# sadhusamik/speech_recognition_tools

Hardware: AMD Instinct MI355X
Metric: audio-hours/sec FDLP featurized (16 kHz, 80-band) (higher is better)
Workload: dtype f64; 1 GPU; wsj_si284_4s_batches; params=wsj, scp_entries_total=1024, batches_in_flight=4, utts_per_batch=1024, nfilters=80, order=150, coeff_num=100, coeff_range=0,100, fbank=cochlear,1,1,1,2.5,1, add_noise=clean, parallelism=scp-shard x1 (contiguous split_scp shards, no collective)

## Files before the change

### speech_recognition_tools_amd/csrc/fdlp_autocorr.hip

```cpp
#include <hip/hip_runtime.h>
#include <math.h>

#include <algorithm>
#include <type_traits>
#include <stdint.h>
#include <stdlib.h>

#include "fdlp_device.h"

namespace fdlp {

constexpr int kAcChunk = 256;
constexpr int kAcRing = 512;
constexpr int kAcPer = kAcChunk / 64;
constexpr int kMaxWrapLags = 256;

template <int NT>
__global__ __launch_bounds__(64, 4) void autocorr_kernel(DevConsts c, const double* __restrict__ dct,
                                                      const double* __restrict__ dense,
                                                      double* __restrict__ rout) {
  static_assert(16 * NT <= kAcChunk, "window halo must fit one chunk");
  constexpr int G = 2;
  constexpr int kEpi = (16 * G + 15) * 17;
  constexpr int kStage = 2 * kAcRing;
  constexpr int kLds = kStage > kEpi ? kStage : kEpi;
  constexpr int NLPL = (16 * NT + 63) / 64;
  __shared__ double xs[kLds];

  const int item = blockIdx.x;
  const int lane = threadIdx.x;
  const int N = c.N;
  int lo, hi;
  const double* drow;
  const double* wrow = nullptr;
  if (dense) {
    lo = 0;
    hi = N;
    drow = dense + (int64_t)item * N;
  } else {
    const int f = item / c.B, j = item % c.B;
    lo = c.lo[j];
    hi = c.hi[j];
    drow = dct + (int64_t)f * N;
    wrow = c.fbank + (int64_t)j * N;
  }
  const int i_lane = lane & 15;
  const int kk_lane = lane >> 4;

  dbl4 acc[NT];
#pragma unroll
  for (int t = 0; t < NT; ++t) acc[t] = dbl4{0.0, 0.0, 0.0, 0.0};

  const int span = hi - lo;
  const int nsteps = (span + 63) / 64;
  const int nchunks = (nsteps + kAcPer - 1) / kAcPer;
  double dv[kAcPer], wv[kAcPer];
  auto fetch = [&](int ch) {
#pragma unroll
    for (int q = 0; q < kAcPer; ++q) {
      int pos = lo + kAcChunk * ch + 64 * q + lane;
      if (pos >= N) pos -= N;
      const bool ok = pos >= lo && pos < hi;
      dv[q] = ok ? drow[pos] : 0.0;
      wv[q] = ok ? (wrow ? wrow[pos] : 1.0) : 0.0;
    }
  };
  auto store = [&](int ch) {
#pragma unroll
    for (int q = 0; q < kAcPer; ++q) {
      const int slot = (kAcChunk * ch + 64 * q + lane) & (kAcRing - 1);
      const double x = wv[q] * dv[q];
      xs[slot] = x;
      xs[slot + kAcRing] = x;
    }
  };
  if (nsteps > 0) {
    fetch(0);
    store(0);
    fetch(1);
    store(1);
    fetch(2);
  }
  __syncthreads();
  for (int ch = 0; ch < nchunks; ++ch) {
    const int s_end = min(kAcPer, nsteps - kAcPer * ch);
    const int rbase = (kAcChunk * ch) & (kAcRing - 1);
    for (int st = 0; st < s_end; ++st) {
      const double* w = xs + rbase + 64 * st + 16 * kk_lane + i_lane;
      const double a = w[0];
#pragma unroll
      for (int t = 0; t < NT; ++t)
        acc[t] = __builtin_amdgcn_mfma_f64_16x16x4f64(a, w[16 * t], acc[t], 0, 0, 0);
    }
    __syncthreads();
    store(ch + 2);
    if (ch + 3 <= nchunks) fetch(ch + 3);
    __syncthreads();
  }

  const int nlags = c.nlags;
  double mine[NLPL];
#pragma unroll
  for (int q = 0; q < NLPL; ++q) mine[q] = 0.0;
  const int col = lane & 15;
  const int row0 = lane >> 4;
#pragma unroll
  for (int tg = 0; tg < NT; tg += G) {
    const int lag_base = 16 * tg - 15;
#pragma unroll
    for (int t = tg; t < tg + G && t < NT; ++t) {
#pragma unroll
      for (int r = 0; r < 4; ++r) {
        const int row = row0 + 4 * r;
        const int lag = 16 * t + col - row;
        xs[(lag - lag_base) * 17 + row] = acc[t][r];
      }
    }
    __syncthreads();
#pragma unroll
    for (int q = 0; q < NLPL; ++q) {
      const int L = lane + 64 * q;
      if (L < nlags && L >= lag_base && L < 16 * (tg + G)) {
        double s = 0.0;
        for (int i = 0; i < 16; ++i) {
          const int t = (L + i) >> 4;
          if (t >= tg && t < tg + G && t < NT) s += xs[(L - lag_base) * 17 + i];
        }
        mine[q] += s;
      }
    }
    __syncthreads();
  }
#pragma unroll
  for (int q = 0; q < NLPL; ++q) {
    const int L = lane + 64 * q;
    if (L < nlags && rout) rout[(int64_t)item * nlags + L] = mine[q];
  }
}


template <int NT, int G, int NLPL>
__device__ __forceinline__ void diag_sums(const dbl4* acc, double* ep, int nlags, int lane, double* mine) {
#pragma unroll
  for (int q = 0; q < NLPL; ++q) mine[q] = 0.0;
  const int col = lane & 15;
  const int row0 = lane >> 4;
#pragma unroll
  for (int tg = 0; tg < NT; tg += G) {
    const int lag_base = 16 * tg - 15;
#pragma unroll
    for (int t = tg; t < tg + G && t < NT; ++t) {
#pragma unroll
      for (int r = 0; r < 4; ++r) {
        const int row = row0 + 4 * r;
        ep[(16 * t + col - row - lag_base) * 17 + row] = acc[t][r];
      }
    }
    __syncthreads();
#pragma unroll
    for (int q = 0; q < NLPL; ++q) {
      const int L = lane + 64 * q;
      if (L < nlags && L >= lag_base && L < 16 * (tg + G)) {
        double s = 0.0;
#pragma unroll
        for (int i = 0; i < 16; ++i) {
          const int t = (L + i) >> 4;
          if (t >= tg && t < tg + G && t < NT) s += ep[(L - lag_base) * 17 + i];
        }
        mine[q] += s;
      }
    }
    __syncthreads();
  }
}

template <int NT, int LB, typename Emit>
__device__ __forceinline__ void diag_blocks(const dbl4* acc, double* ep, int nlags, int lane, Emit emit) {
  static_assert(LB == 32 || LB == 64, "lag block");
  constexpr int LPL = 64 / LB;
  constexpr int TPB = LB / 16;
  constexpr int NB = (16 * NT + LB - 1) / LB;
  const int col = lane & 15;
  const int row0 = lane >> 4;
  const int m = lane / LPL;
  const int part = lane % LPL;
#pragma unroll
  for (int g = 0; g < NB; ++g) {
    if (LB * g >= nlags) break;
#pragma unroll
    for (int u = 0; u <= TPB; ++u) {
      const int t = TPB * g + u;
#pragma unroll
      for (int r = 0; r < 4; ++r) {
        const int row = row0 + 4 * r;
        const double v = t < NT ? acc[t < NT ? t : 0][r] : 0.0;
        ep[(16 * u + col - row + 15) * 17 + row] = v;
      }
    }
    wave_lds_sync();
    const double* src = ep + (m + 15) * 17 + part * (16 / LPL);
    double v[16 / LPL];
#pragma unroll
    for (int i = 0; i < 16 / LPL; ++i) v[i] = src[i];
    double sum = 0.0;
#pragma unroll
    for (int i = 0; i < 16 / LPL; ++i) sum += v[i];
    if constexpr (LPL == 2) sum += dpp_f64<0xB1>(sum);
    const int L = LB * g + m;
    if (part == 0 && L < nlags) {
      if constexpr (std::is_invocable_v<Emit, int, int, double>) emit(g, L, sum);
      else emit(L, sum);
    }
    wave_lds_sync();
  }
}

template <int NT>
__device__ __forceinline__ void lag_step(dbl4* acc, const double* w, bool keep) {
  const double a = keep ? w[0] : 0.0;
#pragma unroll
  for (int t = 0; t < NT; ++t) acc[t] = __builtin_amdgcn_mfma_f64_16x16x4f64(a, w[16 * t], acc[t], 0, 0, 0);
}

template <int NT, int G, bool SNAP = true>
__global__ __launch_bounds__(64, 2) void ac_sweep_kernel(DevConsts c, const double* __restrict__ dct,
                                                         double* __restrict__ rlow, double* __restrict__ rup,
                                                         int nwork) {
  static_assert(16 * NT <= kAcChunk, "window halo must fit one chunk");
  constexpr int kEpi = (G + 31) * 17;
  __shared__ double xs[2 * kAcRing];
  __shared__ double ep[kEpi];

  const int w = xcd_item();
  if (w >= nwork) return;
  const int f = w >> 1;
  const int sk = w & 1;
  const int lane = threadIdx.x;
  const int N = c.N, B = c.B, nlags = c.nlags;
  const double* drow = dct + (int64_t)f * N;
  const double* ew = c.sk_e + (int64_t)sk * N;
  const SkSnap* snaps = c.sk_snap + sk * B;
  double* out = (sk == 0 ? rlow : rup) + (int64_t)f * B * nlags;
  const int T0 = ((N + kAcChunk - 1) / kAcChunk) * kAcChunk;
  const int bmin = c.sk_min[sk] >> 6;
  const int nblk = (T0 >> 6) - bmin;
  const int nchunks = (nblk + kAcPer - 1) / kAcPer;
  const int i_lane = lane & 15;
  const int kk_lane = lane >> 4;

  dbl4 acc[NT];
#pragma unroll
  for (int t = 0; t < NT; ++t) acc[t] = dbl4{0.0, 0.0, 0.0, 0.0};

  double dv[kAcPer], ev[kAcPer];
  auto fetch = [&](int ch) {
#pragma unroll
    for (int q = 0; q < kAcPer; ++q) {
      const int n = T0 - kAcChunk * (ch + 1) + 64 * q + lane;
      const bool ok = n >= 0 && n < N;
      const int m = ok ? (sk == 0 ? N - 1 - n : n) : 0;
      dv[q] = drow[m];
      ev[q] = ok ? ew[m] : 0.0;
    }
  };
  auto store = [&](int ch) {
#pragma unroll
    for (int q = 0; q < kAcPer; ++q) {
      const int slot = (T0 - kAcChunk * (ch + 1) + 64 * q + lane) & (kAcRing - 1);
      const double v = ev[q] * dv[q];
      xs[slot] = v;
      xs[slot + kAcRing] = v;
    }
  };
  extern __shared__ SkSnap tab[];
  for (int q = lane; q < B; q += 64) tab[q] = snaps[q];
  __syncthreads();
  int k = 0;
  SkSnap cur = tab[0];
  auto snapshot = [&]() {
    double* o = out + (int64_t)cur.band * nlags;
    const double K = cur.K;
    if constexpr (SNAP) {
      diag_blocks<NT, G>(acc, ep, nlags, lane, [&](int L, double v) { o[L] = K * v; });
    } else {
      double cs = 0.0;
#pragma unroll
      for (int t = 0; t < NT; ++t) cs += acc[t][0] + acc[t][1] + acc[t][2] + acc[t][3];
      if (lane < nlags) o[lane] = K * cs;
    }
    ++k;
    cur = k < B ? tab[k] : SkSnap{-1, 0, 0.0};
  };
  auto step = [&](int P, int lo, int hi) {
    const int pa = P + 16 * kk_lane + i_lane;
    lag_step<NT>(acc, xs + (P & (kAcRing - 1)) + 16 * kk_lane + i_lane, pa >= lo && pa < hi);
  };

#pragma unroll
  for (int q = 0; q < kAcPer; ++q) {
    const int slot = (T0 + 64 * q + lane) & (kAcRing - 1);
    xs[slot] = 0.0;
    xs[slot + kAcRing] = 0.0;
  }
  fetch(0);
  store(0);
  if (nchunks > 1) fetch(1);
  __syncthreads();
  for (int ch = 0; ch < nchunks; ++ch) {
    for (int q = kAcPer - 1; q >= 0; --q) {
      const int P = T0 - kAcChunk * (ch + 1) + 64 * q;
      if ((P >> 6) < bmin) break;
      int hiM = P + 64;
      while (k < B && cur.S >= hiM) snapshot();
      while (k < B && cur.S > P) {
        step(P, cur.S, hiM);
        hiM = cur.S;
        snapshot();
      }
      step(P, P, hiM);
    }
    __syncthreads();
    if (ch + 1 < nchunks) store(ch + 1);
    if (ch + 2 < nchunks) fetch(ch + 2);
    __syncthreads();
  }
  while (k < B) snapshot();
}

template <int NT, bool VS>
__global__ __launch_bounds__(64, 4) void ac_band_kernel(DevConsts c, const double* __restrict__ dct,
                                                        double* __restrict__ r, const double* __restrict__ rup,
                                                        const double* __restrict__ rflat,
                                                        const double* __restrict__ rpart,
                                                        const double* __restrict__ rwrap, int items) {
  static_assert(16 * NT <= kAcChunk, "window halo must fit one chunk");
  constexpr int kEpi = (32 + 31) * 17;
  constexpr int kWin = (16 * NT + 63) / 64 * 64;
  constexpr int kLds = 2 * kAcRing > kEpi ? 2 * kAcRing : kEpi;
  static_assert(kEpi <= kLds && 2 * kWin + 16 * NT <= kLds, "LDS regions");
  __shared__ double xs[kLds];

  const int item = xcd_item();
  if (item >= items) return;
  const int lane = threadIdx.x;
  const int N = c.N, nlags = c.nlags;
  const int f = item / c.B, j = item % c.B;
  const int2 reg = c.sk_reg[j];
  const int m1 = reg.x, m2 = reg.y;
  FDLP_CHECK(0 <= m1 && m1 <= m2 && m2 <= N && j < c.B);
  const double kw = (VS && rwrap) ? c.sk_wrap[j] : 0.0;
  const double* drow = dct + (int64_t)f * N;
  const double* wrow = c.fbank + (int64_t)j * N;
  const int i_lane = lane & 15;
  const int kk_lane = lane >> 4;

  dbl4 acc[NT];
#pragma unroll
  for (int t = 0; t < NT; ++t) acc[t] = dbl4{0.0, 0.0, 0.0, 0.0};

  if constexpr (!VS) {
    const int lo = m1, hi = m2;
    const int nsteps = (hi - lo + 63) / 64;
    const int nchunks = (nsteps + kAcPer - 1) / kAcPer;
    double dv[kAcPer];
    auto fetch = [&](int ch) {
#pragma unroll
      for (int q = 0; q < kAcPer; ++q) {
        const int pos = lo + kAcChunk * ch + 64 * q + lane;
        dv[q] = pos < hi ? drow[pos] : 0.0;
      }
    };
    auto store = [&](int ch) {
#pragma unroll
      for (int q = 0; q < kAcPer; ++q) {
        const int slot = (kAcChunk * ch + 64 * q + lane) & (kAcRing - 1);
        xs[slot] = dv[q];
        xs[slot + kAcRing] = dv[q];
      }
    };
    if (nsteps > 0) {
      fetch(0);
      store(0);
      fetch(1);
      store(1);
      fetch(2);
    }
    __syncthreads();
    for (int ch = 0; ch < nchunks; ++ch) {
      const int s_end = min(kAcPer, nsteps - kAcPer * ch);
      const int rbase = (kAcChunk * ch) & (kAcRing - 1);
      for (int st = 0; st < s_end; ++st)
        lag_step<NT>(acc, xs + rbase + 64 * st + 16 * kk_lane + i_lane, true);
      __syncthreads();
      store(ch + 2);
      if (ch + 3 <= nchunks) fetch(ch + 3);
      __syncthreads();
    }
  }

  constexpr int kSt = (kWin + 16 * NT + 63) / 64;
  static_assert(kSt > kWin / 64 && kWin % 64 == 0, "window layout");
  auto straddle = [&](const double* xa, const double* xb, int st0) {
#pragma unroll
    for (int st = 0; st < kWin / 64; ++st) {
      if (st < st0) continue;
      const int w = 64 * st + 16 * kk_lane + i_lane;
      const double a = xa[w];
      const int tmin = (kWin - 64 * st - 48) >> 4;
      double bv[NT];
#pragma unroll
      for (int t = 0; t < NT; ++t)
        if (t >= tmin) bv[t] = xb[w + 16 * t];
#pragma unroll
      for (int t = 0; t < NT; ++t)
        if (t >= tmin) acc[t] = __builtin_amdgcn_mfma_f64_16x16x4f64(a, bv[t], acc[t], 0, 0, 0);
    }
  };
  constexpr int kReg = kWin + 64 + 16 * NT;
  constexpr bool kFits = 2 * kReg <= kLds;
#ifdef FDLP_AB_BAND_GENERIC
  const bool fast = false;
#else
  const bool fast = kFits && VS && kw != 0.0 && m1 >= kWin && m2 - m1 >= nlags - 1 && m2 + (kSt * 64 - kWin) <= N;
#endif
  if constexpr (kFits) if (fast) {
    constexpr int kA = kWin / 64, kB = kSt - kWin / 64;
    static_assert(kB <= kA + 1, "m2 B taps");
    double d1[kSt], w1[kA], d2[kSt], w2[kA];
    {
      const double* s1 = drow + (m1 - kWin) + lane;
      const double* t1 = wrow + (m1 - kWin) + lane;
      const double* s2 = drow + (m2 - kWin) + lane;
      const double* t2 = wrow + m2 + lane;
      FDLP_CHECK(m1 - kWin >= 0 && m2 + 64 * kB <= N);
#pragma unroll
      for (int u = 0; u < kSt; ++u) d1[u] = s1[64 * u];
#pragma unroll
      for (int u = 0; u < kA; ++u) w1[u] = t1[64 * u];
#pragma unroll
      for (int u = 0; u < kSt; ++u) d2[u] = s2[64 * u];
#pragma unroll
      for (int u = 0; u < kA; ++u) w2[u] = t2[64 * u];
    }
    double* r1 = xs;
    double* r2 = xs + kReg;
#pragma unroll
    for (int u = 0; u < kA; ++u) {
      r1[64 * u + lane] = w1[u] * d1[u];
      r2[64 * u + lane] = d2[u];
    }
    r1[kWin + lane] = 0.0;
    r2[kWin + lane] = 0.0;
#pragma unroll
    for (int u = 0; u < kB; ++u) {
      const int q = 64 * u + lane;
      if (q < 16 * NT) {
        r1[kWin + 64 + q] = d1[kA + u];
        r2[kWin + 64 + q] = u < kA ? (w2[u] - 1.0) * d2[kA + u] : 0.0;
      }
    }
    __syncthreads();
    straddle(r1, r1 + 64, 0);
    straddle(r2, r2 + 64, 0);
  }
  if (!fast) {
    double* xa = xs;
    double* xb = xs + kWin;
#pragma unroll 1
    for (int e = 0; e < (kw != 0.0 ? 2 : 3); ++e) {
      const int b = e == 0 ? m1 : (e == 1 ? m2 : N);
      int lb = e == 0 ? 0 : (e == 1 ? m1 : m2);
      lb = max(lb, b - (nlags - 1));
      if (lb >= b) continue;
      double wv[kSt], dv[kSt];
#pragma unroll
      for (int u = 0; u < kSt; ++u) {
        const int pos = b - kWin + 64 * u + lane;
        const int pm = pos < 0 ? 0 : (pos >= N ? pos - N : pos);
        FDLP_CHECK(pm >= 0 && pm < N);
        wv[u] = wrow[pm];
        dv[u] = drow[pm];
      }
      __syncthreads();
#pragma unroll
      for (int u = 0; u < kSt; ++u) {
        const int q = 64 * u + lane;
        const int pos = b - kWin + q;
        const double x = pos >= lb ? wv[u] * dv[u] : 0.0;
        if constexpr (VS) {
          if (q < kWin + 16 * NT) xb[q] = pos >= b ? (e == 1 && pos < N ? (wv[u] - 1.0) * dv[u] : x) : 0.0;
        } else {
          if (q < kWin + 16 * NT) xb[q] = pos >= b ? x : 0.0;
        }
        if (q < kWin) xa[q] = pos < b ? x : 0.0;
      }
      __syncthreads();
      straddle(xa, xb, (lb - b + kWin) >> 6);
    }
  }
  __syncthreads();
  double* ro = r + (int64_t)item * nlags;
  const double* uo = rup + (int64_t)item * nlags;
  if constexpr (VS) {
    constexpr int kNB = (16 * NT + 31) / 32;
    double sums[kNB];
#pragma unroll
    for (int g = 0; g < kNB; ++g) sums[g] = 0.0;
    diag_blocks<NT, 32>(acc, xs, nlags, lane, [&](int g, int, double v) { sums[g] = v; });
    const double* fo = rflat + (int64_t)item * nlags;
    const int2 fb = c.fl_band[j];
    const int pmask = fb.y & ((1 << (c.fl_H - 1)) - 1);
    double rv[kNB], uv[kNB], fv[kNB], wv[kNB];
    const double* wo = rwrap + (int64_t)f * nlags;
    static_assert(32 * kNB - (16 * (NT - 1) - 14) <= kRowSlack, "row slack covers the last lag block");
    const int lh = lane >> 1;
    FDLP_CHECK(32 * kNB <= nlags + kRowSlack);
#pragma unroll
    for (int g = 0; g < kNB; ++g) {
      rv[g] = ro[lh + 32 * g];
      uv[g] = uo[lh + 32 * g];
      fv[g] = fo[lh + 32 * g];
      wv[g] = kw != 0.0 ? wo[lh + 32 * g] : 0.0;
    }
    if (pmask) {
      for (int rest = pmask; rest; rest &= rest - 1) {
        FDLP_CHECK(__builtin_ctz(rest) < c.fl_H - 1 && fb.x >= 0 && fb.x < kMaxChains);
        const double* po = rpart + (((int64_t)f * (c.fl_H - 1) + __builtin_ctz(rest)) * kMaxChains + fb.x) * nlags + lh;
#pragma unroll
        for (int g = 0; g < kNB; ++g) fv[g] += po[32 * g];
      }
    }
#pragma unroll
    for (int g = 0; g < kNB; ++g) {
      const int L = 32 * g + (lane >> 1);
      if ((lane & 1) == 0 && L < nlags) {
        const double v = sums[g] + rv[g] + uv[g] + fv[g];
        ro[L] = kw != 0.0 ? v + kw * wv[g] : v;
      }
    }
  } else {
    diag_blocks<NT, 32>(acc, xs, nlags, lane, [&](int L, double v) { ro[L] = v + ro[L] + uo[L]; });
  }
}

__global__ __launch_bounds__(64) void ac_wrap_kernel(DevConsts c, const double* __restrict__ dct,
                                                     double* __restrict__ rwrap, int nframes) {
  __shared__ double zt[kMaxWrapLags], yh[kMaxWrapLags];
  const int f = blockIdx.x;
  if (f >= nframes) return;
  const int N = c.N, nlags = c.nlags, L1 = nlags - 1;
  const double* drow = dct + (int64_t)f * N;
  for (int i = threadIdx.x; i < L1; i += 64) {
    const int mt = N - L1 + i;
    zt[i] = c.sk_e[N + mt] * drow[mt];
    yh[i] = c.sk_e[i] * drow[i];
  }
  __syncthreads();
  for (int l = threadIdx.x; l < nlags; l += 64) {
    double acc = 0.0;
    for (int i = 0; i < l; ++i) acc = fma(zt[L1 - l + i], yh[i], acc);
    rwrap[(int64_t)f * nlags + l] = acc;
  }
}


constexpr int kVsMirror = 16;
template <int C>
constexpr int vs_ring() { return kVsRingPositions; }
template <int C>
constexpr int vs_row() { return 544; }
template <int A, int C>
constexpr int vs_chunk() { return vs_chunk_positions(A, C > 0); }
template <int C>
constexpr int vs_waves_per_simd() { return 2; }

template <int A>
struct VsOrder {
  int v[A * A], u[A * A];
};
template <int A>
constexpr VsOrder<A> vs_order() {
  VsOrder<A> o{};
  int n = 0;
  for (int w = 0; w < A - 1; ++w)
    for (int u = A - 1; u > w; --u) {
      o.v[n] = A + w - u;
      o.u[n] = u;
      ++n;
    }
  for (int q = 0; q < A; ++q)
    for (int u = q; u >= 0; --u) {
      o.v[n] = q - u;
      o.u[n] = u;
      ++n;
    }
  return o;
}
template <int A, int I = 0>
__device__ __forceinline__ void vs_fma_rows(double (&acc)[A], double cur, const double (&lo)[A], const double (&hi)[A]) {
  if constexpr (I < A * A) {
    constexpr VsOrder<A> o = vs_order<A>();
    constexpr int V = o.v[I], U = o.u[I];
    static_assert(V >= 0 && V < A && U >= 0 && U < A, "block order");
    fmac_bcast_ordered<V>(acc[U], cur, (V + U < A) ? lo[V + U] : hi[V + U - A]);
    vs_fma_rows<A, I + 1>(acc, cur, lo, hi);
  }
}
template <int A>
__device__ __forceinline__ void vs_fma_block(double (&acc)[A], double cur, const double (&lo)[A],
                                             const double (&hi)[A]) {
  double cm;
  asm volatile("v_mov_b64 %0, %1\n\ts_nop 1" : "=v"(cm) : "v"(cur));
  vs_fma_rows<A>(acc, cm, lo, hi);
}

template <int A, int C>
__global__ __launch_bounds__(64, vs_waves_per_simd<C>()) void ac_vsweep_kernel(DevConsts c, const double* __restrict__ dct,
                                                          double* __restrict__ rlow, double* __restrict__ rup,
                                                          double* __restrict__ rflat,
                                                          double* __restrict__ rpart,
                                                          const SkSnap* __restrict__ snaps,
                                                          const FlatEv* __restrict__ fev, int nframes,
                                                          int ngroups) {
  constexpr int kVsChunk = vs_chunk<A, C>();
  constexpr int kVsRing = vs_ring<C>();
  constexpr int kRow = vs_row<C>();
  static_assert(A % 2 == 0 && A <= 16 && 18 * A < kVsRing - kVsChunk && A <= kVsMirror + 1, "vsweep geometry");
  static_assert(kRow >= kVsRing + kVsMirror && kVsRing % 2 == 0, "ring row");
  auto slot_of = [](int n) {
    if constexpr ((kVsRing & (kVsRing - 1)) == 0) return n & (kVsRing - 1);
    else return (n + 8 * kVsRing) % kVsRing;
  };
  auto slot_add = [&](int u, int d) {
    if constexpr ((kVsRing & (kVsRing - 1)) == 0) {
      return (u + d) & (kVsRing - 1);
    } else {
      const int b = slot_of(__builtin_amdgcn_readfirstlane(u)) + d;
      return b >= kVsRing ? b - kVsRing : b;
    }
  };
  __shared__ double ring_all[4][kRow];
  static_assert(kVsMirror <= 32, "mirror fits the row padding");
  const int H = C == 0 ? 2 : c.fl_H;
  const int item = xcd_item();
  if (item >= H * ngroups) return;
  const int g = item / H;
  const int part = item - H * g;
  const int kind = C == 0 ? part : 2;
  const int lane = threadIdx.x;
  const int row = lane >> 4;
  const int l = lane & 15;
  const int f = 4 * g + row;
  const bool fvalid = f < nframes;
  const int N = c.N, B = c.B, nlags = c.nlags;
  const double* drow = dct + (int64_t)(fvalid ? f : 0) * N;
  const double* ew = c.sk_e + (int64_t)(kind == 1 ? N : 0);
  double* rg = ring_all[row];
  const int nlo = kind == 2 ? c.fl_part_lo[part] : c.sk_min[kind];
  const int nhi = kind == 2 ? c.fl_part_hi[part] : N;
  const int kbeg = kind == 2 ? c.fl_part_ev[part] : 0;
  const int kend = kind == 2 ? c.fl_part_ev[part + 1] : B;
  auto part_store = [&](auto&& value) {
    if (kind == 2 && part < H - 1) {
      for (int cc = 0; cc < C; ++cc) {
        double* o = rpart + (((int64_t)f * (H - 1) + part) * kMaxChains + cc) * nlags;
#pragma unroll
        for (int u = 0; u < A; ++u)
          if (fvalid && A * l + u < nlags) o[A * l + u] = value(cc, u);
      }
    }
  };
  if (nhi <= nlo) {
    for (int k = kbeg; k < kend; ++k) {
      const int band = kind == 2 ? fev[k].band : snaps[kind * B + k].band;
      if (kind == 2 && fev[k].type == 0) continue;
      double* o = (kind == 0 ? rlow : (kind == 1 ? rup : rflat)) + ((int64_t)f * B + band) * nlags;
#pragma unroll
      for (int u = 0; u < A; ++u)
        if (fvalid && A * l + u < nlags) o[A * l + u] = 0.0;
    }
    part_store([](int, int) { return 0.0; });
    return;
  }

  constexpr int kPf = kVsChunk / 16;
  double pf[kPf], pe[C == 0 ? kPf : 1];
  static_assert((kVsRing & (kVsRing - 1)) == 0 && kVsRing % kVsChunk == 0 && kVsMirror == 16, "aligned chunk runs");
  auto inside = [&](int base) { return C == 0 && base >= 0 && base + kVsChunk <= N; };
  auto issue = [&](int base) __attribute__((always_inline)) {
    if (inside(base)) {
      if (kind == 0) {
        const double* pd = drow + (N - 1 - base - l);
        const double* pw = ew + (N - 1 - base - l);
#pragma unroll
        for (int q = 0; q < kPf; ++q) {
          pf[q] = __builtin_nontemporal_load(pd - 16 * q);
          if constexpr (C == 0) pe[q] = pw[-16 * q];
        }
      } else {
        const double* pd = drow + base + l;
        const double* pw = ew + base + l;
#pragma unroll
        for (int q = 0; q < kPf; ++q) {
          pf[q] = __builtin_nontemporal_load(pd + 16 * q);
          if constexpr (C == 0) pe[q] = pw[16 * q];
        }
      }
    } else {
#pragma unroll
      for (int q = 0; q < kPf; ++q) {
        const int n = min(max(base + 16 * q + l, 0), N - 1);
        const int m = kind == 0 ? N - 1 - n : n;
        pf[q] = __builtin_nontemporal_load(drow + m);
        if constexpr (C == 0) pe[q] = ew[m];
      }
    }
  };
  auto commit = [&](int base) __attribute__((always_inline)) {
    if (inside(base)) {
      const int sb = base & (kVsRing - 1);
      double* w = rg + sb + l;
#pragma unroll
      for (int q = 0; q < kPf; ++q) {
        double v = pf[q];
        if constexpr (C == 0) v = pe[q] * v;
        w[16 * q] = v;
      }
      if (sb == 0) {
        double v = pf[0];
        if constexpr (C == 0) v = pe[0] * v;
        rg[kVsRing + l] = v;
      }
    } else {
#pragma unroll
      for (int q = 0; q < kPf; ++q) {
        const int n = base + 16 * q + l;
        const int slot = slot_add(base, 16 * q + l);
        double v = pf[q];
        if constexpr (C == 0) v = pe[q] * v;
        v = (n >= 0 && n < N) ? v : 0.0;
        FDLP_CHECK(slot >= 0 && slot < kVsRing);
        rg[slot] = v;
        if (slot < kVsMirror) rg[kVsRing + slot] = v;
      }
    }
  };
  const int b_top = (nhi - 1) / A;
  const int b_bot = nlo / A;

  double acc[A];
#pragma unroll
  for (int u = 0; u < A; ++u) acc[u] = 0.0;
  double ch[C > 0 ? C : 1][A];
#pragma unroll
  for (int k = 0; k < (C > 0 ? C : 1); ++k)
#pragma unroll
    for (int u = 0; u < A; ++u) ch[k][u] = 0.0;

  constexpr int P = C == 0 ? 2 : 1;
  double* const outb = kind == 0 ? rlow : (kind == 1 ? rup : rflat);
  double pend[P][A];
  int64_t prow[P];
  int npend = 0;
#pragma unroll
  for (int i = 0; i < P; ++i) {
    prow[i] = 0;
#pragma unroll
    for (int u = 0; u < A; ++u) pend[i][u] = 0.0;
  }
  auto flush = [&]() {
#pragma unroll
    for (int i = 0; i < P; ++i) {
      if (i < npend) {
        double* o = outb + prow[i];
#pragma unroll
        for (int u = 0; u < A; ++u)
          if (fvalid && A * l + u < nlags) o[A * l + u] = pend[i][u];
      }
    }
    npend = 0;
  };
  auto push = [&](const double (&v)[A], double K, int band) {
    if (npend == P) flush();
#pragma unroll
    for (int i = 0; i < P; ++i) {
      if (i == npend) {
#pragma unroll
        for (int u = 0; u < A; ++u) pend[i][u] = K * v[u];
        FDLP_CHECK(band >= 0 && band < B);
        prow[i] = ((int64_t)f * B + band) * nlags;
      }
    }
    ++npend;
  };

  int lo_loaded = ((A * b_top + 17 * A - 1 + kVsChunk - 1) / kVsChunk) * kVsChunk;
  issue(lo_loaded - kVsChunk);
  auto ensure = [&](int n0) __attribute__((always_inline)) {
    while (n0 < lo_loaded) {
      lo_loaded -= kVsChunk;
      commit(lo_loaded);
      flush();
      issue(lo_loaded - kVsChunk);
      wave_lds_sync();
    }
  };
  ensure(A * b_top);

  int k = kbeg;
  typedef int VsRec __attribute__((ext_vector_type(4), aligned(4)));
  static_assert(sizeof(SkSnap) == 16 && sizeof(FlatEv) == 16, "event records are four words");
  int evS = -1, evBand = 0, evW2 = 0, evW3 = 0;
  VsRec nx = {-1, 0, 0, 0};
  bool nxOk = false;
  auto ev_load = [&](int kk) __attribute__((always_inline)) {
    kk = __builtin_amdgcn_readfirstlane(kk);
    nxOk = kk < kend;
    const int ki = max(min(kk, kend - 1), 0);
    if constexpr (C > 0) nx = *reinterpret_cast<const VsRec*>(fev + ki);
    else nx = *reinterpret_cast<const VsRec*>(snaps + __builtin_amdgcn_readfirstlane(kind * B + ki));
  };
  auto ev_next = [&]() __attribute__((always_inline)) {
    evS = nxOk ? nx.x : -1;
    evBand = nx.y, evW2 = nx.z, evW3 = nx.w;
    ev_load(k + 1);
  };
  ev_load(k);
  ev_next();
  auto handle_at = [&](int S) __attribute__((always_inline)) {
    if constexpr (C > 0) {
#pragma unroll
      for (int cc = 0; cc < C; ++cc)
#pragma unroll
        for (int u = 0; u < A; ++u) ch[cc][u] += acc[u];
#pragma unroll
      for (int u = 0; u < A; ++u) acc[u] = 0.0;
    }
    while (evS == S) {
      if constexpr (C > 0) {
#pragma unroll
        for (int cc = 0; cc < C; ++cc) {
          if (cc == evW3) {
            if (evW2 == 1) push(ch[cc], 1.0, evBand);
#pragma unroll
            for (int u = 0; u < A; ++u) ch[cc][u] = evW2 == 0 ? 0.0 : ch[cc][u];
          }
        }
      } else {
        push(acc, __hiloint2double(__builtin_amdgcn_readfirstlane(evW3), __builtin_amdgcn_readfirstlane(evW2)), evBand);
      }
      ++k;
      ev_next();
    }
  };

  static_assert(19 * A < kVsRing - kVsChunk, "ring room for staging one block ahead");
  double cur_ahead = rg[slot_add(A * b_top, l)];
  auto block = [&](int n0, double (&lo)[A], const double (&hi)[A]) {
    const int n1 = max(n0 - A, A * b_bot);
    ensure(n1);
    asm volatile("" ::"s"(nx));
    asm volatile("" : "+v"(cur_ahead));
    const int base = slot_add(n0, A * l);
    FDLP_CHECK(base >= 0 && base + A <= kVsRing + kVsMirror);
#pragma unroll
    for (int q = 0; q < A; ++q) lo[q] = rg[base + q];
    const double cur = cur_ahead;
    cur_ahead = rg[slot_add(n1, l)];
    const int pos = n0 + l;
    int hi_m = min(n0 + A, nhi);
    for (;;) {
      while (evS >= hi_m) handle_at(evS);
      const int lo_m = max(max(evS, n0), nlo);
      vs_fma_block<A>(acc, (pos >= lo_m && pos < hi_m) ? cur : 0.0, lo, hi);
      if (lo_m <= n0 || lo_m <= nlo) break;
      hi_m = lo_m;
    }
  };

  double X[A], Y[A];
  {
    const int base = slot_add(A * b_top + A, A * l);
#pragma unroll
    for (int q = 0; q < A; ++q) Y[q] = rg[base + q];
  }
  auto plain = [&](int n0, double (&lo)[A], const double (&hi)[A]) __attribute__((always_inline)) {
    FDLP_CHECK(evS < n0 && n0 >= nlo && n0 + A <= nhi && n0 - A >= A * b_bot);
    FDLP_CHECK(n0 - A >= lo_loaded && n0 + 16 * A <= lo_loaded + kVsRing);
    const int base = slot_add(n0, A * l);
#pragma unroll
    for (int q = 0; q < A; ++q) lo[q] = rg[base + q];
    const double cur = cur_ahead;
    cur_ahead = rg[slot_add(n0 - A, l)];
    vs_fma_block<A>(acc, cur, lo, hi);
  };
  const int b_whole = vs_whole_top(nhi, A);
  for (int b = b_top; b >= b_bot;) {
#pragma unroll 1
    for (int m = vs_run_pairs(b, b_whole, evS, lo_loaded, b_bot, A); m > 0; --m) {
      plain(A * b, X, Y);
      plain(A * b - A, Y, X);
      b -= 2;
    }
    block(A * b, X, Y);
    if (--b < b_bot) break;
    block(A * b, Y, X);
    --b;
  }
  while (k < kend) handle_at(evS);
  flush();
  if constexpr (C > 0) {
    part_store([&](int cc, int u) {
      double v = 0.0;
#pragma unroll
      for (int q = 0; q < C; ++q)
        if (q == cc) v = ch[q][u] + acc[u];
      return v;
    });
  }
#pragma unroll
  for (int i = 0; i < P; ++i)
#pragma unroll
    for (int u = 0; u < A; ++u) asm volatile("" ::"v"(pend[i][u]));
}


template <int NT>
static hipError_t launch_ac_nt(const DevConsts& c, const double* dct, const double* dense, int items,
                               double* r, hipStream_t s) {
  hipLaunchKernelGGL((autocorr_kernel<NT>), dim3(items), dim3(64), 0, s, c, dct, dense, r);
  (void)kmark(kKAutocorr, s);
  return hipGetLastError();
}

int autocorr_tiles(int nlags) { return ((nlags + 14) >> 4) + 1; }

static hipError_t launch_autocorr_any(const DevConsts& c, const double* dct, const double* dense, int items,
                                      double* r, hipStream_t s) {
  if (items <= 0) return hipSuccess;
  switch (autocorr_tiles(c.nlags)) {
#define FDLP_AC_CASE(n) case n: return launch_ac_nt<n>(c, dct, dense, items, r, s);
    FDLP_AC_CASE(1) FDLP_AC_CASE(2) FDLP_AC_CASE(3) FDLP_AC_CASE(4) FDLP_AC_CASE(5)
    FDLP_AC_CASE(6) FDLP_AC_CASE(7) FDLP_AC_CASE(8) FDLP_AC_CASE(9) FDLP_AC_CASE(10)
    FDLP_AC_CASE(11) FDLP_AC_CASE(12) FDLP_AC_CASE(13) FDLP_AC_CASE(14) FDLP_AC_CASE(15)
    FDLP_AC_CASE(16)
#undef FDLP_AC_CASE
    default: return hipErrorInvalidValue;
  }
}

hipError_t launch_autocorr(const DevConsts& c, const double* dct, const double* dense, int items,
                           double* r, hipStream_t s) {
  return launch_autocorr_any(c, dct, dense, items, r, s);
}

int vsweep_lanes_lags(int nlags) {
  const int a = (nlags + 15) / 16;
  for (int v : {4, 8, 10})
    if (a <= v) return v;
  return 0;
}
int vsweep_chains(int C) {
  for (int v : {4, 5, 6, 8})
    if (C <= v) return v;
  return 0;
}

template <int A, int C>
static hipError_t launch_vsweep_ac(const DevConsts& c, const double* dct, int nframes, double* r, double* rup,
                                   double* rflat, double* rpart, hipStream_t s) {
  const int ngroups = (nframes + 3) / 4;
  hipLaunchKernelGGL((ac_vsweep_kernel<A, 0>), dim3(xcd_grid(2 * ngroups)), dim3(64), 0, s, c, dct, r, rup, rflat,
                     rpart, c.sk_snap, c.fl_ev, nframes, ngroups);
  (void)kmark(kKVsweepSkirt, s);
  hipLaunchKernelGGL((ac_vsweep_kernel<A, C>), dim3(xcd_grid(c.fl_H * ngroups)), dim3(64), 0, s, c, dct, r, rup,
                     rflat, rpart, c.sk_snap, c.fl_ev, nframes, ngroups);
  (void)kmark(kKVsweepFlat, s);
  return hipGetLastError();
}
template <int A>
static hipError_t launch_vsweep_a(const DevConsts& c, const double* dct, int nframes, double* r, double* rup,
                                  double* rflat, double* rpart, hipStream_t s) {
  switch (vsweep_chains(c.fl_C)) {
    case 4: return launch_vsweep_ac<A, 4>(c, dct, nframes, r, rup, rflat, rpart, s);
    case 5: return launch_vsweep_ac<A, 5>(c, dct, nframes, r, rup, rflat, rpart, s);
    case 6: return launch_vsweep_ac<A, 6>(c, dct, nframes, r, rup, rflat, rpart, s);
    case 8: return launch_vsweep_ac<A, 8>(c, dct, nframes, r, rup, rflat, rpart, s);
    default: return hipErrorInvalidValue;
  }
}
static hipError_t launch_vsweep(const DevConsts& c, const double* dct, int nframes, double* r, double* rup,
                                double* rflat, double* rpart, hipStream_t s) {
  switch (vsweep_lanes_lags(c.nlags)) {
    case 4: return launch_vsweep_a<4>(c, dct, nframes, r, rup, rflat, rpart, s);
    case 8: return launch_vsweep_a<8>(c, dct, nframes, r, rup, rflat, rpart, s);
    case 10: return launch_vsweep_a<10>(c, dct, nframes, r, rup, rflat, rpart, s);
    default: return hipErrorInvalidValue;
  }
}

template <int NT>
static hipError_t launch_struct_nt(const DevConsts& c, const double* dct, int nframes, double* r, double* rup,
                                   double* rflat, double* rpart, double* rwrap, hipStream_t s) {
  if (rflat) {
    const hipError_t e = launch_vsweep(c, dct, nframes, r, rup, rflat, rpart, s);
    if (e != hipSuccess) return e;
    const bool wrap = rwrap && c.sk_wrap && c.nlags <= kMaxWrapLags;
    if (wrap) {
      hipLaunchKernelGGL(ac_wrap_kernel, dim3(nframes), dim3(64), 0, s, c, dct, rwrap, nframes);
      (void)kmark(kKAcWrap, s);
    }
    hipLaunchKernelGGL((ac_band_kernel<NT, true>), dim3(xcd_grid(nframes * c.B)), dim3(64), 0, s, c, dct, r, rup,
                       rflat, rpart, wrap ? rwrap : nullptr, nframes * c.B);
    (void)kmark(kKAcBand, s);
    return hipGetLastError();
  }
  const size_t tab = sizeof(SkSnap) * (size_t)c.B;
  hipLaunchKernelGGL((ac_sweep_kernel<NT, 32>), dim3(xcd_grid(2 * nframes)), dim3(64), tab, s, c, dct, r, rup, 2 * nframes);
  (void)kmark(kKAcSweep, s);
  hipLaunchKernelGGL((ac_band_kernel<NT, false>), dim3(xcd_grid(nframes * c.B)), dim3(64), 0, s, c, dct, r, rup,
                     nullptr, nullptr, nullptr, nframes * c.B);
  (void)kmark(kKAcBand, s);
  return hipGetLastError();
}

hipError_t launch_autocorr_structured(const DevConsts& c, const double* dct, int nframes, double* r,
                                      double* rup, double* rflat, double* rpart, double* rwrap, hipStream_t s) {
  if (nframes <= 0) return hipSuccess;
  if (!c.sk_e || !c.sk_snap || !c.sk_reg) return hipErrorInvalidValue;
  if (rflat && (!c.fl_ev || !c.fl_band || (c.fl_H > 1 && !rpart))) return hipErrorInvalidValue;
  switch (autocorr_tiles(c.nlags)) {
#define FDLP_ST_CASE(n) case n: return launch_struct_nt<n>(c, dct, nframes, r, rup, rflat, rpart, rwrap, s);
    FDLP_ST_CASE(1) FDLP_ST_CASE(2) FDLP_ST_CASE(3) FDLP_ST_CASE(4) FDLP_ST_CASE(5)
    FDLP_ST_CASE(6) FDLP_ST_CASE(7) FDLP_ST_CASE(8) FDLP_ST_CASE(9) FDLP_ST_CASE(10)
    FDLP_ST_CASE(11) FDLP_ST_CASE(12) FDLP_ST_CASE(13) FDLP_ST_CASE(14) FDLP_ST_CASE(15)
    FDLP_ST_CASE(16)
#undef FDLP_ST_CASE
    default: return hipErrorInvalidValue;
  }
}

hipError_t checks_autocorr(unsigned int* v, bool reset) { return fdlp_checks_local(v, reset); }

}
```

Measured before the change: 242.4 audio-hours/s.

## Use a 2x2 fast-product reformulation in the autocorrelation vsweep inner loop

```diff
diff --git a/speech_recognition_tools_amd/csrc/fdlp_autocorr.hip b/speech_recognition_tools_amd/csrc/fdlp_autocorr.hip
--- a/speech_recognition_tools_amd/csrc/fdlp_autocorr.hip
+++ b/speech_recognition_tools_amd/csrc/fdlp_autocorr.hip
@@ -613,6 +613,50 @@
   asm volatile("v_mov_b64 %0, %1\n\ts_nop 1" : "=v"(cm) : "v"(cur));
   vs_fma_rows<A>(acc, cm, lo, hi);
 }
+
+template <int A>
+struct VsBank22 {
+  double e[A], od[A / 2], w0;
+};
+template <int A>
+struct VsOrder22 {
+  static constexpr int kN = 3 * (A / 2) * (A / 2);
+  int src[kN], v[kN], acc[kN], op[kN], nold;
+};
+template <int A>
+constexpr VsOrder22<A> vs_order22() {
+  VsOrder22<A> o{};
+  int n = 0;
+  for (int pass = 0; pass < 2; ++pass) {
+    for (int t = pass == 0 ? A : 0; t <= (pass == 0 ? 2 * A - 4 : A - 2); t += 2) {
+      const int umax = t < A - 2 ? t : A - 2, umin = t - (A - 2) > 0 ? t - (A - 2) : 0;
+      for (int u = umax; u >= umin; u -= 2) o.src[n] = 0, o.v[n] = t - u, o.acc[n] = u, o.op[n] = t, ++n;
+      for (int u = umax; u >= umin; u -= 2) o.src[n] = 1, o.v[n] = t - u, o.acc[n] = u / 2, o.op[n] = t + 1, ++n;
+      for (int u = umax; u >= umin; u -= 2) o.src[n] = 0, o.v[n] = t - u + 1, o.acc[n] = u + 1, o.op[n] = t + 1, ++n;
+    }
+    if (pass == 0) o.nold = n;
+  }
+  return o;
+}
+template <int A, int I, int END>
+__device__ __forceinline__ void vs_fma22(double (&acc)[A], double (&M)[A / 2], double cm, double csm,
+                                         const VsBank22<A>& lo, const VsBank22<A>& hi) {
+  if constexpr (I < END) {
+    constexpr VsOrder22<A> o = vs_order22<A>();
+    constexpr int V = o.v[I], U = o.acc[I], W = o.op[I];
+    static_assert(V >= 0 && V < A && W >= 0 && W < 2 * A - 2, "block order");
+    if constexpr (o.src[I] == 0) {
+      static_assert(U < A, "block order");
+      fmac_bcast_ordered<V>(acc[U], cm, W < A ? lo.e[W] : hi.e[W - A]);
+    } else {
+      static_assert(U < A / 2 && (W & 1) == 1 && (V & 1) == 0, "block order");
+      fmac_bcast_ordered<V>(M[U], csm, W < A ? lo.od[W / 2] : hi.od[(W - A) / 2]);
+    }
+    vs_fma22<A, I + 1, END>(acc, M, cm, csm, lo, hi);
+  }
+}
+template <int A, int C>
+constexpr bool vs_fast22() { return !(A == 8 && C == 4) && !(A == 10 && C >= 6); }
 
 template <int A, int C>
 __global__ __launch_bounds__(64, vs_waves_per_simd<C>()) void ac_vsweep_kernel(DevConsts c, const double* __restrict__ dct,
@@ -896,11 +940,69 @@
   };
   const int b_whole = vs_whole_top(nhi, A);
   for (int b = b_top; b >= b_bot;) {
+    if constexpr (vs_fast22<A, C>()) {
+      int m = vs_run_pairs(b, b_whole, evS, lo_loaded, b_bot, A);
+      if (m > 0) {
+        double cur1_ahead = rg[slot_add(A * b, l) + 1];
+        VsBank22<A> bx, by;
+#pragma unroll
+        for (int q = 0; q + 1 < A; ++q) by.e[q] = (q & 1) ? Y[q + 1] - Y[q] : Y[q] - Y[q + 1];
+        by.e[A - 1] = 0.0;
+#pragma unroll
+        for (int q = 0; q < A / 2; ++q) by.od[q] = Y[2 * q + 1];
+        by.w0 = Y[0];
+        double M[A / 2];
+#pragma unroll
+        for (int q = 0; q < A / 2; ++q) M[q] = 0.0;
+        auto plain22 = [&](int n0, VsBank22<A>& lo, const VsBank22<A>& hi) __attribute__((always_inline)) {
+          FDLP_CHECK(evS < n0 && n0 >= nlo && n0 + A <= nhi && n0 - A >= A * b_bot);
+          FDLP_CHECK(n0 - A >= lo_loaded && n0 + 16 * A <= lo_loaded + kVsRing);
+          FDLP_CHECK(n0 - A + 1 >= lo_loaded && n0 - A + 1 + 15 < lo_loaded + kVsRing);
+          FDLP_CHECK(slot_add(n0 - A, l) + 1 < kVsRing + kVsMirror);
+          const int base = slot_add(n0, A * l);
+          double w[A];
+#pragma unroll
+          for (int q = 0; q < A; ++q) w[q] = rg[base + q];
+          const double cur = cur_ahead, curs = cur_ahead + cur1_ahead;
+          const int ahead = slot_add(n0 - A, l);
+          cur_ahead = rg[ahead];
+          cur1_ahead = rg[ahead + 1];
+          double cm, csm;
+          asm volatile("v_mov_b64 %0, %2\n\tv_mov_b64 %1, %3\n\ts_nop 1" : "=&v"(cm), "=&v"(csm) : "v"(cur), "v"(curs));
+          constexpr int kOld = vs_order22<A>().nold;
+          vs_fma22<A, 0, kOld>(acc, M, cm, csm, lo, hi);
+#pragma unroll
+          for (int q = 0; q < A; ++q) asm volatile("" : "+v"(w[q]));
+#pragma unroll
+          for (int q = 0; q + 1 < A; ++q) lo.e[q] = (q & 1) ? w[q + 1] - w[q] : w[q] - w[q + 1];
+          lo.e[A - 1] = hi.w0 - w[A - 1];
+#pragma unroll
+          for (int q = 0; q < A / 2; ++q) lo.od[q] = w[2 * q + 1];
+          lo.w0 = w[0];
+          vs_fma22<A, kOld, VsOrder22<A>::kN>(acc, M, cm, csm, lo, hi);
+        };
 #pragma unroll 1
-    for (int m = vs_run_pairs(b, b_whole, evS, lo_loaded, b_bot, A); m > 0; --m) {
-      plain(A * b, X, Y);
-      plain(A * b - A, Y, X);
-      b -= 2;
+        for (; m > 0; --m) {
+          plain22(A * b, bx, by);
+          plain22(A * b - A, by, bx);
+          b -= 2;
+        }
+#pragma unroll
+        for (int u = 0; u < A; ++u) acc[u] += M[u >> 1];
+        const int n0 = A * b + A;
+        FDLP_CHECK(n0 >= lo_loaded && n0 + 16 * A <= lo_loaded + kVsRing);
+        const int base = slot_add(n0, A * l);
+        FDLP_CHECK(base >= 0 && base + A <= kVsRing + kVsMirror);
+#pragma unroll
+        for (int q = 0; q < A; ++q) Y[q] = rg[base + q];
+      }
+    } else {
+#pragma unroll 1
+      for (int m = vs_run_pairs(b, b_whole, evS, lo_loaded, b_bot, A); m > 0; --m) {
+        plain(A * b, X, Y);
+        plain(A * b - A, Y, X);
+        b -= 2;
+      }
     }
     block(A * b, X, Y);
     if (--b < b_bot) break;
```

Measured after the change: 250.4 audio-hours/s, median of 6. +3.3%, better.
